# Mikata-Project/adcraft

Hardware: AMD Instinct MI355X
Metric: env-steps/sec (envs×keywords auctions/s) (higher is better)
Workload: dtype i32 cents + f32 (Philox4x32-7 u32); 1 GPU; cfg2: 4096 envs x 256 keywords per GPU, IMPLICIT keywords, mean_volume 128, cvr 0.8, no_vol_prob 0.0, drift False, budget non-binding, 60-step episodes with auto-reset; envs_per_gpu=4096, keywords=256, parallelism=env-sharded x1, collective=none (single GPU), weak_scaling_reference=also.cfg4.value of the N=1 --full line (same per-GPU shard as the N>1 runs)

## Files before the change

### adcraft_amd/_ffi.py

```python
import ctypes as C
import os

from . import build as _build

ADC_OK, ADC_EINVAL, ADC_EHIP, ADC_ENOMEM, ADC_ESTATE, ADC_ETYPE, ADC_ERCCL = 0, -1, -2, -3, -4, -5, -6
MODEL_IMPLICIT, MODEL_EXPLICIT, MODEL_IMPLICIT_GENERAL = 0, 1, 2
P_VOL_MEAN, P_VOL_STD, P_A, P_B, P_BCTR, P_SCTR, P_REV_MEAN, P_REV_STD, P_COUNT = range(9)
(BUF_PARAMS, BUF_BIDS, BUF_BUDGET, BUF_IMPRESSIONS, BUF_CLICKS, BUF_CONVERSIONS, BUF_COST, BUF_REVENUE, BUF_REWARD,
 BUF_CUM_PROFIT, BUF_DAYS, BUF_TERMINATED, BUF_TRUNCATED, BUF_METRIC_PROFIT, BUF_METRIC_SCALARS, BUF_FLAT_OBS,
 BUF_ROLLOUT_ACTION, BUF_ROLLOUT_LOGP, BUF_ROLLOUT_VALUE, BUF_ROLLOUT_REWARD, BUF_ROLLOUT_TERMINATED, BUF_ROLLOUT_TRUNCATED,
 BUF_ROLLOUT_OBS) = range(23)
MLP_TANH, MLP_RELU = 0, 1
ES_CENTERED_RANK, ES_RAW = 0, 1
ES_ADAM, ES_SGD = 0, 1
ROLLOUT_OBS = 1
PG_ADAM, PG_SGD = 0, 1
TD3_ADAM, TD3_SGD = 0, 1
PBT_PG, PBT_TD3 = 0, 1


class EngineError(RuntimeError):
    pass


# ... 161 lines not shown
        "adc_engine_set_env_drift": ([vp, vp], C.c_int),
        "adc_engine_get_rng_state": ([vp, vp, vp], C.c_int),
        "adc_engine_set_rng_state": ([vp, vp, vp], C.c_int),
        "adc_engine_get_episode_state": ([vp, vp, vp], C.c_int),
        "adc_engine_set_episode_state": ([vp, vp, vp], C.c_int),
        "adc_engine_step": ([vp, vp, vp, C.POINTER(StepOut)], C.c_int),
        "adc_engine_step_device": ([vp, vp, vp], C.c_int),
        "adc_engine_step_async": ([vp, vp, vp, C.POINTER(StepOut)], C.c_int),
        "adc_engine_step_flat_async": ([vp, vp, vp, vp, vp, vp], C.c_int),
        "adc_engine_wait": ([vp], C.c_int),
        "adc_engine_fetch": ([vp, C.POINTER(StepOut)], C.c_int),
        "adc_engine_out_offsets": ([vp, C.POINTER(C.c_size_t), C.POINTER(C.c_size_t)], C.c_int),
        "adc_engine_synchronize": ([vp], C.c_int),
        "adc_engine_step_flat": ([vp, vp, vp, vp, vp, vp], C.c_int),
        "adc_engine_step_replay": ([vp, vp, vp, C.POINTER(Tape), C.POINTER(StepOut)], C.c_int),
        "adc_engine_update_keywords": ([vp], C.c_int),
        "adc_engine_set_general_model": ([vp, i32, f32, i32], C.c_int),
        "adc_host_alloc": ([C.c_size_t, C.POINTER(vp)], C.c_int),
        "adc_host_free": ([vp], None),
        "adc_engine_device_buffer": ([vp, C.c_int, C.POINTER(vp), C.POINTER(C.c_size_t)], C.c_int),
        "adc_engine_stream": ([vp, C.POINTER(vp)], C.c_int),
        "adc_engine_sample_actions": ([vp, f32, f32, f32], C.c_int),
        "adc_engine_set_flat_actions_device": ([vp, vp], C.c_int),
        "adc_engine_flat_obs_enable": ([vp, C.c_int], C.c_int),
        "adc_engine_profile_enable": ([vp, C.c_int], C.c_int),
        "adc_engine_profile_sample_every": ([vp, C.c_int32], C.c_int),
        "adc_engine_profile_read": ([vp, vp, C.POINTER(i64)], C.c_int),
        "adc_engine_profile_records": ([vp, C.POINTER(i64)], C.c_int),
        "adc_engine_region_begin": ([vp], C.c_int),
        "adc_engine_region_end": ([vp, C.POINTER(f64)], C.c_int),
        "adc_engine_comm_stats": ([vp, C.POINTER(i64), C.POINTER(f64), C.POINTER(f64), C.c_int], C.c_int),
        "adc_engine_step_kernel_name": ([vp], C.c_char_p),
        "adc_engine_metrics_enable": ([vp, C.c_int], C.c_int),
        "adc_engine_metrics_reset": ([vp], C.c_int),
        "adc_engine_metrics_read": ([vp, vp, vp], C.c_int),
        "adc_engine_ideal_profit": ([vp, C.c_int, vp, C.c_int, vp], C.c_int),
        "adc_bid_curves_from_samples": ([C.c_int, vp, i32, vp, i32, vp, vp], C.c_int),
        "adc_engine_metrics_akncp_ncp": ([vp, f64, vp, vp], C.c_int),
        "adc_engine_bid_curves_contenders": ([vp, vp, vp, C.POINTER(i32)], C.c_int),
        "adc_engine_outcomes_replay": ([vp, i32, i32, vp, f32, i64, vp, vp, vp, vp, C.POINTER(i64), vp], C.c_int),
        "adc_engine_outcomes_replay_tape": ([vp, i32, vp, f32, C.POINTER(Tape), i64, vp, vp, vp, vp, C.POINTER(i64), vp], C.c_int),
        "adc_nth_price_auction": ([C.c_int, f64, vp, i32, i32, i32, i32, C.POINTER(i32), vp, vp], C.c_int),
        "adc_sigmoid": ([f64, f64, f64], f64),
        "adc_clamp": ([f64, f64, f64], f64),
        "adc_threshold_sigmoid": ([f64, f64, f64, f64], f64),
        "adc_sum_f64": ([vp, i64], f64),
        "adc_count_true": ([vp, i64], i64),
        "adc_nonneg_int_normal": ([f64, f64, u64, u64], u64),
        "adc_binomial": ([u64, f64, u64, u64], u64),
        "adc_cost_create": ([f64, i64, u64, u64, vp], C.c_int),
        "adc_auction_word_intervals": ([f32, f32, f32, f32, vp], C.c_int),
        "adc_auction_word_brackets": ([f32, f32, f32, f32, vp], C.c_int),
        "adc_check_win_brackets": ([i64, vp, vp, vp, vp, vp, vp, vp], i64),
        "adc_sample_random_keyword": ([C.c_uint64, C.c_uint32, C.c_uint32, vp], C.c_int),
        "adc_interp_act_host": ([f32, i32, f32, i32, C.c_double, C.c_double, C.c_double, vp, i32, i32, vp, vp, i32, vp, vp,
                                 C.c_double, vp, vp, vp, vp, vp], C.c_int),
        "adc_interp_key_host": ([f32], C.c_double),
        "adc_engine_mlp_init": ([vp, C.POINTER(MLPConfig), vp], C.c_int),
        "adc_engine_mlp_set_layer": ([vp, i32, i32, vp, vp], C.c_int),
        "adc_engine_mlp_set_norm": ([vp, vp, vp], C.c_int),
        "adc_engine_mlp_set_log_std": ([vp, vp], C.c_int),
        "adc_engine_mlp_set_deterministic": ([vp, i32], C.c_int),
        "adc_engine_mlp_act": ([vp, f32, vp], C.c_int),
        "adc_engine_mlp_step": ([vp, f32], C.c_int),
        "adc_engine_mlp_last": ([vp, vp, vp, vp, vp, vp], C.c_int),
        "adc_engine_mlp_bootstrap_value": ([vp, vp], C.c_int),
        "adc_engine_mlp_agent_state": ([vp, vp, vp], C.c_int),
        "adc_engine_rollout_enable": ([vp, i32, i32], C.c_int),
        "adc_engine_rollout_reset": ([vp], C.c_int),
        "adc_engine_rollout_fetch": ([vp, C.POINTER(i32), vp, vp, vp, vp, vp, vp, vp], C.c_int),
        "adc_engine_mlp_population": ([vp, i32, vp], C.c_int),
        "adc_engine_mlp_set_member_layer": ([vp, i32, i32, vp, vp], C.c_int),
        "adc_engine_mlp_param_count": ([vp, C.POINTER(i64)], C.c_int),
        "adc_engine_mlp_get_params": ([vp, vp], C.c_int),
        "adc_engine_mlp_get_member_params": ([vp, i32, vp], C.c_int),
        "adc_engine_mlp_learners": ([vp, i32], C.c_int),
        "adc_engine_mlp_set_learner_layer": ([vp, i32, i32, i32, vp, vp], C.c_int),
        "adc_engine_mlp_set_learner_log_std": ([vp, i32, vp], C.c_int),
        "adc_engine_mlp_get_learner_params": ([vp, i32, vp], C.c_int),
        "adc_engine_es_init": ([vp, C.POINTER(ESConfig)], C.c_int),
        "adc_engine_es_perturb": ([vp], C.c_int),
        "adc_engine_es_fitness": ([vp, vp], C.c_int),
        "adc_engine_es_update": ([vp, vp, C.POINTER(ESStats)], C.c_int),
        "adc_engine_es_state_get": ([vp, vp, vp, vp, C.POINTER(i64)], C.c_int),
        "adc_engine_es_state_set": ([vp, vp, vp, vp, i64], C.c_int),
        "adc_es_config_check": ([C.POINTER(ESConfig), C.POINTER(C.c_char_p)], C.c_int),
        "adc_es_noise_host": ([u64, C.c_uint32, C.c_uint32, i64, i64, vp], C.c_int),
        "adc_es_update_host": ([C.POINTER(ESConfig), u64, i32, i64, vp, i64, vp, vp, vp, vp], C.c_int),
        "adc_engine_pg_init": ([vp, C.POINTER(PGConfig)], C.c_int),
        "adc_engine_pg_param_count": ([vp, C.POINTER(i64)], C.c_int),
        "adc_engine_pg_advantages": ([vp], C.c_int),
        "adc_engine_pg_advantages_fetch": ([vp, vp, vp], C.c_int),
        "adc_engine_pg_minibatch": ([vp, i32, i32, C.POINTER(PGStats)], C.c_int),
        "adc_engine_pg_update": ([vp, i32, C.POINTER(PGStats)], C.c_int),
        "adc_engine_pg_state_get": ([vp, vp, vp, vp, C.POINTER(i64)], C.c_int),
        "adc_engine_pg_state_set": ([vp, vp, vp, vp, i64], C.c_int),
        "adc_pg_pop_config_check": ([C.POINTER(PGConfig), i32, i32, i32, C.POINTER(C.c_char_p)], C.c_int),
        "adc_engine_pg_pop_init": ([vp, C.POINTER(PGConfig), i32], C.c_int),
        "adc_engine_pg_pop_advantages": ([vp], C.c_int),
        "adc_engine_pg_pop_advantages_fetch": ([vp, vp, vp], C.c_int),
        "adc_engine_pg_pop_minibatch": ([vp, i32, C.POINTER(PGStats)], C.c_int),
        "adc_engine_pg_pop_update": ([vp, i32, C.POINTER(PGStats)], C.c_int),
        "adc_engine_pg_pop_state_get": ([vp, i32, vp, vp, vp, C.POINTER(i64)], C.c_int),
        "adc_engine_pg_pop_state_set": ([vp, i32, vp, vp, vp, i64], C.c_int),
        "adc_engine_pg_pop_set_config": ([vp, i32, C.POINTER(PGConfig)], C.c_int),
        "adc_engine_pg_pop_copy": ([vp, i32, i32], C.c_int),
# ... 141 lines not shown
```

### adcraft_amd/csrc/adc_law.h

```cpp
#pragma once
#include <stdint.h>

#if defined(__HIPCC__)
#include <hip/hip_runtime.h>
#define ADC_HD __host__ __device__ __forceinline__
#else
#include <math.h>
#define ADC_HD static inline
#endif

namespace adc {

enum Stage : uint32_t { ST_VOL = 0, ST_AUCTION = 1, ST_DRIFT = 2, ST_XPHANTOM = 3, ST_XREV = 4, ST_ACTION = 5, ST_METRIC = 6, ST_CONV = 7, ST_KEYGEN = 8, ST_AGENT = 9,
                        ST_GBIDDERS = 10, ST_GBID = 11, ST_GCLICK = 12, ST_INTERP = 13, ST_MLP = 14 };
constexpr int kTimesteps = 24;
constexpr int kVolumeMax = 1 << 20;
constexpr float kMoneyMaxCents = 1.0e9f;

struct U4 { uint32_t x, y, z, w; };

ADC_HD uint32_t xor3(uint32_t a, uint32_t b, uint32_t c)
{
#if defined(__HIP_DEVICE_COMPILE__)
    return __builtin_amdgcn_bitop3_b32(a, b, c, 0x96);
// ... 311 lines not shown
template <typename Tab>
ADC_HD float laplace_deviate_from_v(uint32_t v24, Tab tab)
{
    const uint32_t neg_mask = 0u - (v24 >> 23);
    const uint32_t mag = (v24 ^ neg_mask) & 0x007FFFFFu;
    const float e = neg_log_f24(fma32((float)mag, 2.0f, 1.0f), tab);
    return bits_to_float(xor_and(float_to_bits(-e), neg_mask, 0x80000000u));
}

template <typename Tab>
ADC_HD int32_t signed_cents_from_v(uint32_t v24, float loc, float scale, Tab tab)
{
    const float x = fma32(__builtin_fabsf(scale), laplace_deviate_from_v(v24, tab), loc);
    float c = __builtin_rintf(x * 100.0f);
    c = c < kMoneyMaxCents ? c : kMoneyMaxCents;
    c = c > -kMoneyMaxCents ? c : -kMoneyMaxCents;
    return (int32_t)c;
}

template <typename Tab>
ADC_HD int32_t competitor_cents_from_v(uint32_t v24, float loc, float scale, Tab tab)
{
    const float x = fma32(__builtin_fabsf(scale), laplace_deviate_from_v(v24, tab), loc);
    float c = __builtin_rintf(__builtin_fabsf(x) * 100.0f);
    c = c < kMoneyMaxCents ? c : kMoneyMaxCents;
    return (int32_t)c;
}

ADC_HD uint32_t auction_uniform24(uint32_t w, const AuctionLaw &a, bool &click)
{
    click = bernoulli32(w, a.t32);
    const uint32_t d = click ? w : w - a.t32;
    const uint32_t v = mulhi32(d, click ? a.m_click : a.m_noclick);
    return v < 0x00FFFFFFu ? v : 0x00FFFFFFu;
}

ADC_HD bool auction_wins(uint32_t w, int32_t bid_c, int32_t comp_c) { return bid_c > comp_c && w != 0xFFFFFFFFu; }

template <typename Tab>
ADC_HD int32_t auction_outcome_unless_top_word(uint32_t w, const AuctionLaw &a, float loc, float scale, Tab tab, bool &click)
{
    click = w < a.t32;
    const uint32_t d = click ? w : w - a.t32;
    const uint32_t v = mulhi32(d, click ? a.m_click : a.m_noclick);
    return competitor_cents_from_v(v < 0x00FFFFFFu ? v : 0x00FFFFFFu, loc, scale, tab);
}

ADC_HD int32_t auction_outcome(uint32_t w, const AuctionLaw &a, float loc, float scale, const LogTableEntry *tab, bool &click)
{
    return competitor_cents_from_v(auction_uniform24(w, a, click), loc, scale, tab);
}


ADC_HD uint32_t lower_bound_v(int32_t target, float loc, float scale, const LogTableEntry *tab)
{
    const float s = __builtin_fabsf(scale);
    const float x_t = ((float)target - 0.5f) * 0.01f;
    const float z_t = (x_t - loc) / s;
    const float e_t = __builtin_fabsf(z_t);
#if defined(__HIP_DEVICE_COMPILE__)
    float mag_f = __builtin_amdgcn_exp2f(fma32(e_t, -1.44269504f, 23.0f));
#else
    float mag_f = exp2f(fma32(e_t, -1.44269504f, 23.0f));
#endif
    mag_f = mag_f < 8388607.0f ? mag_f : 8388607.0f;
    mag_f = mag_f > 0.0f ? mag_f : 0.0f;
    const uint32_t mag = (uint32_t)mag_f;
    const uint32_t est = z_t < 0.0f ? mag : 0x00FFFFFFu - mag;
    float slack = mag_f * (6.0e-6f + 2.4e-7f * (__builtin_fabsf(x_t) + __builtin_fabsf(loc)) / s);
    slack = slack < 4194304.0f ? slack : 4194304.0f;
    const uint32_t half = 8u + (uint32_t)slack;
    uint32_t lo = est > half ? est - half : 0u;
    uint32_t hi = est + half < 0x01000000u ? est + half : 0x01000000u;
    if (lo > 0u && !(signed_cents_from_v(lo - 1u, loc, scale, tab) < target)) lo = 0u;
    if (hi < 0x01000000u && !(signed_cents_from_v(hi, loc, scale, tab) >= target)) hi = 0x01000000u;
    while (lo < hi) {
        const uint32_t mid = (lo + hi) >> 1;
        if (signed_cents_from_v(mid, loc, scale, tab) >= target) hi = mid;
        else lo = mid + 1u;
    }
    return lo;
}

ADC_HD uint64_t offset_reaching(uint32_t W, uint32_t m, uint64_t range)
{
    if (W == 0u) return 0ull;
    if (W > 0x00FFFFFFu || m == 0u) return range;
    const double q = ((double)W * 4294967296.0) / (double)m;
    if (!(q < (double)range)) return range;
    uint64_t d = (uint64_t)q;
    const uint64_t need = (uint64_t)W << 32;
    if (d * m >= need) { if (d > 0ull && (d - 1ull) * m >= need) d -= 1ull; }
    else { d += 1ull; if (d * m < need) d += 1ull; }
    return d < range ? d : range;
}

struct WinIntervals { uint32_t c_lo, c_w, n_lo, n_w; };

ADC_HD WinIntervals win_intervals(int32_t bid_c, float loc, float scale, uint64_t t_click, const AuctionLaw &law, const LogTableEntry *tab)
{
    const uint32_t w_lo = lower_bound_v(1 - bid_c, loc, scale, tab);
    const uint32_t w_hi = lower_bound_v(bid_c, loc, scale, tab);
    WinIntervals r{0u, 0u, 0u, 0u};
    if (!(w_lo < w_hi)) return r;
    const uint64_t top = 0xFFFFFFFFull;
    uint64_t a = offset_reaching(w_lo, law.m_click, t_click), b = offset_reaching(w_hi, law.m_click, t_click);
    b = b < top ? b : top;
    if (a < b) { r.c_lo = (uint32_t)a; r.c_w = (uint32_t)(b - a); }
    const uint64_t range_n = 4294967296ull - t_click;
    a = t_click + offset_reaching(w_lo, law.m_noclick, range_n);
    b = t_click + offset_reaching(w_hi, law.m_noclick, range_n);
    b = b < top ? b : top;
    if (a < b) { r.n_lo = (uint32_t)a; r.n_w = (uint32_t)(b - a); }
    return r;
}

struct WinBrackets { WinIntervals out, in; };
constexpr float kWordSlack = 4096.0f;

ADC_HD float fast_exp2(float x)
{
#if defined(__HIP_DEVICE_COMPILE__)
    return __builtin_amdgcn_exp2f(x);
#else
    return exp2f(x);
#endif
}
ADC_HD float fast_rcp(float x)
{
#if defined(__HIP_DEVICE_COMPILE__)
    return __builtin_amdgcn_rcpf(x);
#else
    return 1.0f / x;
#endif
}
ADC_HD float min_num(float a, float b) { return __builtin_fminf(a, b); }
ADC_HD float max_num(float a, float b) { return __builtin_fmaxf(a, b); }
ADC_HD uint32_t sat_sub(uint32_t a, uint32_t b)
{
#if defined(__clang__)
    return __builtin_elementwise_sub_sat(a, b);
#else
    return a > b ? a - b : 0u;
#endif
}
ADC_HD uint32_t to_word(float x)
{
#if defined(__HIP_DEVICE_COMPILE__)
    return (uint32_t)x;
#else
    return !(x > 0.0f) ? 0u : x >= 4294967296.0f ? 0xFFFFFFFFu : (uint32_t)x;
#endif
}

ADC_HD void lower_bound_estimate(float x_t, float loc, float inv_s, float &est, float &slack)
{
    const float z_t = (x_t - loc) * inv_s;
    const float e_t = __builtin_fabsf(z_t);
    const float mag = min_num(fast_exp2(fma32(e_t, -1.44269504f, 23.0f)), 8388607.0f);
    est = z_t < 0.0f ? mag : 16777215.0f - mag;
    const float rel = fma32(1.0e-6f, fma32(__builtin_fabsf(x_t) + __builtin_fabsf(loc), inv_s, e_t), 2.0e-5f);
    slack = min_num(fma32(mag, rel, 16.0f), 33554432.0f);
}

ADC_HD WinBrackets win_brackets(int32_t bid_c, float loc, float scale, float t_f)
{
    const float inv_s = fast_rcp(__builtin_fabsf(scale));
    const float bc = (float)bid_c;
    float lo, lo_s, hi, hi_s;
    lower_bound_estimate(fma32(bc, -0.01f, 0.005f), loc, inv_s, lo, lo_s);
    lower_bound_estimate(fma32(bc, 0.01f, -0.005f), loc, inv_s, hi, hi_s);
    const float lo_out = lo - lo_s, lo_in = lo + lo_s, hi_out = hi + hi_s, hi_in = hi - hi_s;
    const float a_c = max_num(t_f * 5.9604644775390625e-08f, 1.0f);
    const float a_n = max_num((4294967296.0f - t_f) * 5.9604644775390625e-08f, 1.0f);
    const float t_dn = t_f - kWordSlack, t_up = t_f + kWordSlack;
    WinBrackets r;
    const uint32_t c_lo_out = to_word(fma32(lo_out, a_c, -kWordSlack)), c_hi_out = to_word(min_num(fma32(hi_out, a_c, kWordSlack), t_f));
    const uint32_t c_lo_in = to_word(fma32(lo_in, a_c, kWordSlack)), c_hi_in = to_word(min_num(fma32(hi_in, a_c, -kWordSlack), t_f));
    const uint32_t n_lo_out = to_word(fma32(lo_out, a_n, t_dn)), n_hi_out = to_word(fma32(hi_out, a_n, t_up));
    const uint32_t n_lo_in = to_word(fma32(lo_in, a_n, t_up)), n_hi_in = to_word(fma32(hi_in, a_n, t_dn));
    r.out = WinIntervals{c_lo_out, sat_sub(c_hi_out, c_lo_out), n_lo_out, sat_sub(n_hi_out, n_lo_out)};
    r.in = WinIntervals{c_lo_in, sat_sub(c_hi_in, c_lo_in), n_lo_in, sat_sub(n_hi_in, n_lo_in)};
    return r;
}

ADC_HD void clicked_win_interval(int32_t bid_c, float loc, float scale, uint64_t t_click, const AuctionLaw &law, const LogTableEntry *tab,
                                 uint32_t &lo, uint32_t &width)
{
    lo = 0u;
    width = 0u;
    const uint32_t w_lo = lower_bound_v(1 - bid_c, loc, scale, tab), w_hi = lower_bound_v(bid_c, loc, scale, tab);
    if (!(w_lo < w_hi)) return;
    const uint64_t a = offset_reaching(w_lo, law.m_click, t_click);
    uint64_t b = offset_reaching(w_hi, law.m_click, t_click);
    b = b < 0xFFFFFFFFull ? b : 0xFFFFFFFFull;
    if (a < b) { lo = (uint32_t)a; width = (uint32_t)(b - a); }
}

ADC_HD int32_t revenue_cents_tab(uint32_t w, float mu, float sd, const NormTableEntry *tab)
{
    float x = fma32(sd, normal_tab(w, tab), mu);
    x = x > 0.01f ? x : 0.01f;
    return money_to_cents(x);
}

ADC_HD int32_t revenue_cents(uint32_t w, float mu, float sd)
{
    float x = fma32(sd, normal_from_word(w), mu);
    x = x > 0.01f ? x : 0.01f;
    return money_to_cents(x);
}

ADC_HD int32_t volume_from_word(uint32_t w, float mean, float sd, const NormTableEntry *tab)
{
    float x = fma32(sd, normal_tab(w, tab), mean);
    x = x > 0.0f ? x : 0.0f;
    x = x < (float)kVolumeMax ? x : (float)kVolumeMax;
    const float t = __builtin_truncf(x);
    return (int32_t)t + ((x - t) >= 0.5f ? 1 : 0);
}

ADC_HD int64_t bid_to_cents(float bid)
{
    double c = __builtin_rint((double)bid * 100.0);
    if (!(c >= 1.0)) c = 1.0;
    if (c > 1.0e9) c = 1.0e9;
    return (int64_t)c;
}
ADC_HD int32_t bid_to_cents_i32(float bid)
{
    double c = __builtin_rint((double)bid * 100.0);
    if (!(c >= 1.0)) c = 1.0;
    if (c > 1.0e9) c = 1.0e9;
    return (int32_t)c;
}
ADC_HD int64_t budget_to_cents(float budget)
{
    double c = __builtin_rint((double)budget * 100.0);
    if (!(c > -9.0e15)) c = -9.0e15;
    if (c > 9.0e15) c = 9.0e15;
    return (int64_t)c;
}

ADC_HD double cents_to_dollars_f64(int cents)
// ... 272 lines not shown
```

### adcraft_amd/csrc/adc_shims.cpp

```cpp
#include <algorithm>
#include <cmath>
#include <cstdint>
#include <thread>
#include <vector>

#include "../../include/adcraft_engine.h"
#include "adc_law.h"
#include "adc_interp.h"
#include "adc_mlp.h"
#include "adc_es.h"
#include "adc_pg.h"
#include "adc_td3.h"
#include "adc_pbt.h"
#include "adc_norm.h"
#include "adc_rew_norm.h"
#include "adc_td3_norm.h"

#define ADC_EXPORT extern "C" __attribute__((visibility("default")))

ADC_EXPORT double adc_sigmoid(double x, double s, double t) { return 1.0 / (1.0 + std::exp(-s * (x - t))); }

ADC_EXPORT double adc_clamp(double x, double lo, double hi) { return x < lo ? lo : (x > hi ? hi : x); }

ADC_EXPORT double adc_threshold_sigmoid(double p, double impression_thresh, double impression_bid_intercept,
// ... 71 lines not shown
{
    if (!out4) return ADC_EINVAL;
    const adc::LogTableEntry *table = host_log_table();
    const adc::AuctionLaw law = adc::make_auction_law(buyside_ctr);
    const adc::WinIntervals r = adc::win_intervals((int32_t)adc::bid_to_cents(bid), cost_loc, cost_scale,
                                                   adc::bernoulli_threshold(buyside_ctr), law, table);
    out4[0] = r.c_lo; out4[1] = r.c_w; out4[2] = r.n_lo; out4[3] = r.n_w;
    return ADC_OK;
}

ADC_EXPORT int adc_auction_word_brackets(float bid, float cost_loc, float cost_scale, float buyside_ctr, uint32_t *out8)
{
    if (!out8) return ADC_EINVAL;
    const adc::WinBrackets b = adc::win_brackets((int32_t)adc::bid_to_cents(bid), cost_loc, cost_scale, adc::bernoulli_threshold_f32(buyside_ctr));
    out8[0] = b.out.c_lo; out8[1] = b.out.c_w; out8[2] = b.out.n_lo; out8[3] = b.out.n_w;
    out8[4] = b.in.c_lo; out8[5] = b.in.c_w; out8[6] = b.in.n_lo; out8[7] = b.in.n_w;
    return ADC_OK;
}

static inline bool interval_inside(uint32_t a_lo, uint32_t a_w, uint32_t b_lo, uint32_t b_w)
{
    if (a_w == 0u) return true;
    return b_w != 0u && a_lo >= b_lo && (uint64_t)a_lo + a_w <= (uint64_t)b_lo + b_w;
}

ADC_EXPORT int64_t adc_check_win_brackets(int64_t n, const float *bid, const float *cost_loc, const float *cost_scale, const float *buyside_ctr,
                                          const uint32_t *brackets8, int64_t *first_bad, double *ambiguous_words)
{
    if (n < 0 || !bid || !cost_loc || !cost_scale || !buyside_ctr) return -1;
    const adc::LogTableEntry *table = host_log_table();
    int64_t bad = 0, first = -1;
    double amb = 0.0;
    for (int64_t i = 0; i < n; ++i) {
        const int32_t bid_c = (int32_t)adc::bid_to_cents(bid[i]);
        const adc::AuctionLaw law = adc::make_auction_law(buyside_ctr[i]);
        const adc::WinIntervals x = adc::win_intervals(bid_c, cost_loc[i], cost_scale[i], adc::bernoulli_threshold(buyside_ctr[i]), law, table);
        adc::WinBrackets b;
        if (brackets8) {
            const uint32_t *p = brackets8 + 8 * i;
            b.out = adc::WinIntervals{p[0], p[1], p[2], p[3]};
            b.in = adc::WinIntervals{p[4], p[5], p[6], p[7]};
        } else {
            b = adc::win_brackets(bid_c, cost_loc[i], cost_scale[i], adc::bernoulli_threshold_f32(buyside_ctr[i]));
        }
        const bool ok = interval_inside(b.in.c_lo, b.in.c_w, x.c_lo, x.c_w) && interval_inside(x.c_lo, x.c_w, b.out.c_lo, b.out.c_w) &&
                        interval_inside(b.in.n_lo, b.in.n_w, x.n_lo, x.n_w) && interval_inside(x.n_lo, x.n_w, b.out.n_lo, b.out.n_w) &&
                        (uint64_t)b.out.c_lo + b.out.c_w <= 0xFFFFFFFFull && (uint64_t)b.out.n_lo + b.out.n_w <= 0xFFFFFFFFull;
        if (!ok) { if (first < 0) first = i; ++bad; }
        amb += ((double)b.out.c_w - (double)b.in.c_w) + ((double)b.out.n_w - (double)b.in.n_w);
    }
    if (first_bad) *first_bad = first;
    if (ambiguous_words) *ambiguous_words = amb;
    return bad;
}

ADC_EXPORT int adc_sample_random_keyword(uint64_t key, uint32_t keyword, uint32_t serial, float *out8)
{
    if (!out8) return ADC_EINVAL;
    adc::generate_explicit_keyword(key, keyword, serial, out8);
    return ADC_OK;
}

ADC_EXPORT int adc_explicit_curve_host(uint64_t key, uint32_t tick, int32_t keyword, int32_t n_samples, float impression_thresh, float a,
                                       float b, const double *bid_grid, int32_t n_bids, double *ir_out, double *cpc_out, double *z_mid2_out)
{
    if (n_samples <= 0 || n_samples > (1 << 20) || keyword < 0 || n_bids < 0 || (n_bids > 0 && (!bid_grid || !ir_out || !cpc_out)))
        return ADC_EINVAL;
    std::vector<float> z((size_t)n_samples);
    for (int32_t i = 0; i < n_samples; i += 4) {
        const adc::U4 w = adc::draw(key, (uint32_t)(i / 4), adc::ST_METRIC, (uint32_t)keyword, tick);
        const uint32_t ws[4] = {w.x, w.y, w.z, w.w};
        for (int j = 0; j < 4 && i + j < n_samples; ++j) z[(size_t)(i + j)] = adc::normal_from_word(ws[j]);
    }
    std::sort(z.begin(), z.end());
    const float z_lo = z[(size_t)((n_samples - 1) / 2)], z_hi = z[(size_t)(n_samples / 2)];
    if (z_mid2_out) { z_mid2_out[0] = z_lo; z_mid2_out[1] = z_hi; }
    for (int32_t i = 0; i < n_bids; ++i) {
        double mu, sigma;
        adc::explicit_cost_law(bid_grid[i], mu, sigma);
        const adc::CurvePoint q = adc::explicit_curve_point(impression_thresh, a, b, z_lo, z_hi, bid_grid[i], mu, sigma);
        ir_out[i] = q.ir;
        cpc_out[i] = q.cpc;
    }
    return ADC_OK;
}

ADC_EXPORT double adc_interp_key_host(float bid) { return adc::interp_key(bid); }

ADC_EXPORT int adc_interp_act_host(float ave_rpc, int32_t n_rpc, float ave_sctr, int32_t n_sctr, double max_observed, double threshold,
                                   double bid_step, const double *grid, int32_t n_bids, int32_t n_clk, const uint16_t *clk_cent,
                                   const float *clk_ave, int32_t n_cpc, const uint16_t *cpc_cent, const double *cpc_ave, double u,
                                   double *margin_out, double *cost_out, double *bid_out, int32_t *index_out,
                                   double *mass_out)
{
    if (n_bids < 1 || n_bids > adc::kInterpMaxBids || !grid || n_clk < 0 || n_cpc < 0 || n_clk > adc::kInterpCents ||
        n_cpc > n_clk || (n_clk > 0 && (!clk_cent || !clk_ave)) || (n_cpc > 0 && (!cpc_cent || !cpc_ave)) || !bid_out || !index_out)
        return ADC_EINVAL;
    for (int i = 0; i < n_clk; ++i)
        if (clk_cent[i] < 1 || clk_cent[i] > adc::kInterpCents || (i > 0 && clk_cent[i] <= clk_cent[i - 1])) return ADC_EINVAL;
    for (int i = 0; i < n_cpc; ++i)
        if (cpc_cent[i] < 1 || cpc_cent[i] > adc::kInterpCents || (i > 0 && cpc_cent[i] <= cpc_cent[i - 1])) return ADC_EINVAL;
    const adc::InterpSeries<float> clk{clk_cent, clk_ave, 1, n_clk};
    const adc::InterpSeries<double> cpc{cpc_cent, cpc_ave, 1, n_cpc};
    double cpc_right = 0.0;
    for (int i = 0; i < n_cpc; ++i) cpc_right = (i == 0 || cpc_ave[i] > cpc_right) ? cpc_ave[i] : cpc_right;
    const double erpc = adc::interp_erpc(ave_rpc, n_rpc, ave_sctr, n_sctr);
// ... 812 lines not shown
```

### adcraft_amd/csrc/parts/kernel_exact_rows.inc

```
#ifdef ADC_EXP_TIMING
#define DBG_T() wall_clock64()
#define DBG_ADD(i, x) dbg[i] += (x)
#else
#define DBG_T() 0ull
#define DBG_ADD(i, x) (void)0
#endif
constexpr int kRowsBlock = 256;
#ifndef ADC_ROWS_MIN_BLOCKS
#define ADC_ROWS_MIN_BLOCKS 4
#endif
constexpr int kRowsMinBlocks = ADC_ROWS_MIN_BLOCKS;
#ifndef ADC_ROWS_MIN_BLOCKS_ONE
#define ADC_ROWS_MIN_BLOCKS_ONE 6
#endif
constexpr int kRowsMinBlocksOne = ADC_ROWS_MIN_BLOCKS_ONE;
constexpr int kRowsMaxK = 2048;
constexpr int kRowsRing = 128;

struct CellStat {
    unsigned int wins, clicks, first;
    unsigned int mask;
    unsigned long long total;
    double sum_d;
    unsigned long long q4;
// ... 637 lines not shown
    __syncthreads();
    if (tid == 0 && !handed) {
        long long profit_c = 0;
        for (int i = 0; i < BLOCK / kWave; ++i) profit_c += rs.wave_part[i];
        exact_pass_epilogue(v, env, hint_in, few_clicks, was_binding, bound_t);
        step_tail(v, env, tick, true, profit_c, 0.0);
    }
    __syncthreads();
    if (tid == 0) rs.cur = (int)gridDim.x + atomicAdd(&v.flag_next[parity], 1);
    __syncthreads();
    fi = rs.cur;
    DBG_ADD(4, 1);
  }
#ifdef ADC_EXP_TIMING
  if (tid == 0) for (int i = 0; i < 8; ++i) atomicAdd(&g_dbg[i], dbg[i]);
#endif
}


#ifdef ADC_EXP_TIMING
__device__ unsigned long long g_rest_phase[20];
#define RDBG_ADD(slot, val) do { if (tid == 0) atomicAdd(&g_rest_phase[slot], (unsigned long long)(val)); } while (0)
#define RDBG_MAX(slot, val) do { if (tid == 0) atomicMax(&g_rest_phase[slot], (unsigned long long)(val)); } while (0)
#else
#define RDBG_ADD(slot, val) (void)0
#define RDBG_MAX(slot, val) (void)0
#endif
constexpr int kRestMaxK = 1024;
struct RestShared {
    long long wave_part[kRowsMaxWaves];
    long long f_R;
    double f_rd;
    int stop_cell;
    int cur;
    int mark_cnt[1][kRowsMaxWaves];
};
constexpr int kRestMarks = 1024;
__host__ __device__ inline size_t rest_lds_bytes(int K) { return (size_t)K * (adc::kTimesteps * 2 + 2 * 8 + 3 * 4); }

struct RestLaws { adc::WinIntervals iv, cheap; adc::AuctionLaw law; float loc, scale; int vol, j_from; };
__device__ __forceinline__ RestLaws rest_laws(const View &v, const float *__restrict__ bids, int env, int K, const RestState &st, int k)
{
    RestLaws L;
    const size_t o = (size_t)env * K + k;
    L.vol = (int)v.rest_counts[o].w;
    int32_t n_unused;
    if (st.row < adc::kTimesteps) adc::cell_range(L.vol, st.row, L.j_from, n_unused);
    else L.j_from = L.vol;
    const int bid_c = (int)adc::bid_to_cents(bids[o]);
    L.loc = param_at(v, ADC_P_A, env, k);
    L.scale = param_at(v, ADC_P_B, env, k);
    const float bctr = param_at(v, ADC_P_BCTR, env, k);
    L.law = adc::make_auction_law(bctr);
    L.iv = adc::win_intervals(bid_c, L.loc, L.scale, adc::bernoulli_threshold(bctr), L.law, g_log_table);
    const int cheap_bid = min(bid_c, (int)(st.R < 0x3FFFFFFFll ? (st.R > 0 ? st.R : 0) : 0x3FFFFFFFll) + 1);
    L.cheap = adc::win_brackets(cheap_bid, L.loc, L.scale, adc::bernoulli_threshold_f32(bctr)).out;
    return L;
}
__device__ __forceinline__ unsigned int rest_count_wins(uint64_t key, uint32_t tick, int K, int k, const RestLaws &L, int a, int b, unsigned short *table)
{
    unsigned int w_count = 0u;
    int last_cw = -1;
    auto one = [&](uint32_t word, int j) {
        const bool cw = (word - L.iv.c_lo) < L.iv.c_w;
        w_count += (unsigned int)(cw | ((word - L.iv.n_lo) < L.iv.n_w));
        if (table && cw && (word - L.cheap.c_lo) < L.cheap.c_w) {
            const int s24 = L.vol / adc::kTimesteps, first24 = L.vol - (adc::kTimesteps - 1) * s24;
            const int row = j < first24 ? 0 : min(1 + (j - first24) / max(s24, 1), adc::kTimesteps - 1);
            const int row_start = row == 0 ? 0 : first24 + (row - 1) * s24;
            if (last_cw < row_start) {
                bool click_bit;
                const int comp = adc::auction_outcome(word, L.law, L.loc, L.scale, g_log_table, click_bit);
                table[row * K + k] = (unsigned short)min(comp, 0xFFFE);
            }
        }
        last_cw = cw ? j : last_cw;
    };
    for (int q = a >> 2; 4 * q < b; ++q) {
        const adc::U4 w = adc::draw(key, (uint32_t)q, adc::ST_AUCTION, (uint32_t)k, tick);
        if (4 * q >= a && 4 * q + 4 <= b) {
            one(w.x, 4 * q); one(w.y, 4 * q + 1); one(w.z, 4 * q + 2); one(w.w, 4 * q + 3);
        } else {
#pragma unroll
            for (int h = 0; h < 4; ++h) {
                const int j = 4 * q + h;
                if (j >= a && j < b) one(h == 0 ? w.x : h == 1 ? w.y : h == 2 ? w.z : w.w, j);
            }
        }
    }
    return w_count;
}

constexpr int kRestPassBlocks = 6;
#ifndef ADC_REST_FRESH_BLOCKS
#define ADC_REST_FRESH_BLOCKS 5
#endif
constexpr int kRestFreshBlocks = ADC_REST_FRESH_BLOCKS;
template <bool PASS_ONLY, bool FRESH = false, int BLOCK = kRowsBlock>
__global__ __launch_bounds__(BLOCK, BLOCK == 512 ? 6 : FRESH ? kRestFreshBlocks : PASS_ONLY ? kRestPassBlocks : 5) void k_step_rest_of_day(View v, const float *__restrict__ bids, int parity)
{
    static_assert(PASS_ONLY || !FRESH, "the at-once variant hands its marks to k_rest_walk");
    static_assert(BLOCK == kRowsBlock || (PASS_ONLY && !FRESH), "wider workgroups: the plain pass only");
    extern __shared__ __align__(16) unsigned char rest_raw[];
    __shared__ RestShared sh;
    const int K = v.K;
    unsigned long long *const a_cost = reinterpret_cast<unsigned long long *>(rest_raw);
    unsigned long long *const a_rev = a_cost + K;
// ... 582 lines not shown
```

### include/adcraft_engine.h

```cpp
#ifndef ADCRAFT_ENGINE_H
#define ADCRAFT_ENGINE_H

#include <stddef.h>
#include <stdint.h>

#ifdef __cplusplus
extern "C" {
#endif

#define ADC_ABI_VERSION 5
#define ADC_STREAM_REVISION 5

typedef enum adc_status {
    ADC_OK = 0,
    ADC_EINVAL = -1,
    ADC_EHIP = -2,
    ADC_ENOMEM = -3,
    ADC_ESTATE = -4,
    ADC_ETYPE = -5,
    ADC_ERCCL = -6
} adc_status;

typedef enum adc_model {
    ADC_MODEL_IMPLICIT = 0,
// ... 446 lines not shown
int adc_pg_gae_norm_host(const adc_pg_config *cfg, int32_t days, int32_t num_envs, const float *reward_tn, const uint8_t *terminated_tn,
                         const uint8_t *truncated_tn, const float *value_tn, const float *bootstrap_n, const float *scale_n, float clip,
                         float *adv_tn, float *ret_tn);

typedef struct adc_td3_norm_config {
    uint32_t struct_size;
    int32_t observations, rewards;
    int32_t per_member;
    double obs_min_std;
    int64_t obs_count_cap;
    double rew_min_std;
    int64_t rew_count_cap;
    float rew_clip;
} adc_td3_norm_config;
int adc_td3_norm_config_check(const adc_td3_norm_config *cfg, const char **message);
int adc_engine_td3_norm_init(adc_engine *e, const adc_td3_norm_config *cfg);
int adc_engine_td3_norm_update(adc_engine *e, int64_t *samples);
int adc_engine_td3_norm_state_get(adc_engine *e, int32_t member, int64_t *obs_count, double *obs_mean_d, double *obs_m2_d, float *shift_d, float *scale_d,
                                  int64_t *rew_count, double *rew_mean, double *rew_m2, float *rew_scale);
int adc_engine_td3_norm_state_set(adc_engine *e, int32_t member, int64_t obs_count, const double *obs_mean_d, const double *obs_m2_d, const float *shift_d,
                                  const float *scale_d, int64_t rew_count, double rew_mean, double rew_m2, float rew_scale);
int adc_engine_td3_norm_returns_get(adc_engine *e, double *g_n);
int adc_engine_td3_norm_returns_set(adc_engine *e, const double *g_n);
int adc_engine_td3_norm_copy(adc_engine *e, const int32_t *src_of_member_m);
int adc_td3_norm_obs_host(const adc_td3_norm_config *cfg, int64_t S, int32_t D, const float *x_sd, int64_t *count, double *mean_d, double *m2_d,
                          float *shift_d, float *scale_d);
int adc_td3_norm_rew_host(const adc_td3_norm_config *cfg, int32_t days, int32_t num_envs, const float *gamma_n, const float *reward_tn,
                          const uint8_t *terminated_tn, const uint8_t *truncated_tn, int64_t *count, double *mean, double *m2, float *scale,
                          double *carry_n);
int adc_td3_y_norm_host(const adc_td3_config *td3, int32_t count, const float *r_b, const uint8_t *done_b, const float *q_b, float scale, float clip,
                        float *y_b);

int adc_engine_outcomes_replay(adc_engine *e, int32_t env, int32_t steps_back, const float *bids_k, float budget, int64_t capacity,
                               int32_t *keyword, int32_t *timestep, double *cost, double *revenue, int64_t *count, int32_t *share_volume_k);
int adc_engine_outcomes_replay_tape(adc_engine *e, int32_t env, const float *bids_k, float budget, const adc_tape *tape, int64_t capacity,
                                    int32_t *keyword, int32_t *timestep, double *cost, double *revenue, int64_t *count, int32_t *share_volume_k);

int adc_nth_price_auction(int device_id, double bid, const double *other_bids, int32_t n_auctions, int32_t n_bidders,
                          int32_t n, int32_t num_winners, int32_t *impressions, int32_t *placements, double *costs);

double adc_sigmoid(double x, double s, double t);
double adc_clamp(double x, double lo, double hi);
double adc_threshold_sigmoid(double p, double impression_thresh,
                             double impression_bid_intercept, double impression_slope);
double adc_sum_f64(const double *x, int64_t n);
int64_t adc_count_true(const uint8_t *x, int64_t n);
uint64_t adc_nonneg_int_normal(double mean, double std, uint64_t seed, uint64_t counter);
uint64_t adc_binomial(uint64_t n, double p, uint64_t seed, uint64_t counter);
int adc_cost_create(double x, int64_t n, uint64_t seed, uint64_t counter, double *out_n);
int adc_auction_word_intervals(float bid, float cost_loc, float cost_scale, float buyside_ctr, uint32_t *out4);
int adc_auction_word_brackets(float bid, float cost_loc, float cost_scale, float buyside_ctr, uint32_t *out8);
int64_t adc_check_win_brackets(int64_t n, const float *bid, const float *cost_loc, const float *cost_scale, const float *buyside_ctr,
                               const uint32_t *brackets8, int64_t *first_bad, double *ambiguous_words);
int adc_sample_random_keyword(uint64_t key, uint32_t keyword, uint32_t serial, float *out8);
int adc_explicit_curve_host(uint64_t key, uint32_t tick, int32_t keyword, int32_t n_samples, float impression_thresh, float a, float b,
                            const double *bid_grid, int32_t n_bids, double *ir_out, double *cpc_out, double *z_mid2_out);
int adc_interp_act_host(float ave_rpc, int32_t num_rpc_obs, float ave_sctr, int32_t num_sctr_obs, double max_observed,
                        double profit_acquisition_threshold, double bid_step, const double *allowed_bids, int32_t n_bids,
                        int32_t n_clicks, const uint16_t *clicks_cent, const float *ave_clicks, int32_t n_cpc, const uint16_t *cpc_cent,
                        const double *ave_cpc, double u, double *margin_out, double *cost_out, double *bid_out, int32_t *index_out,
                        double *mass_out);
double adc_interp_key_host(float bid);
int adc_mlp_act_host(const adc_mlp_config *cfg, int32_t num_keywords, const float *obs_d, const float *const *policy_w,
                     const float *const *policy_b, const float *const *value_w, const float *const *value_b, const float *shift_d,
                     const float *scale_d, const float *log_std_a, const float *normals_a, uint64_t agent_key, uint32_t tick,
                     float budget_override, float *mean_a, float *log_std_out_a, float *action_a, float *logp, float *value,
                     float *bids_k, float *budget);
int adc_es_config_check(const adc_es_config *cfg, const char **message);
int adc_es_noise_host(uint64_t seed, uint32_t pair, uint32_t generation, int64_t p0, int64_t n, float *eps_n);
int adc_es_update_host(const adc_es_config *cfg, uint64_t seed, int32_t members, int64_t n_params, const double *fitness_m, int64_t generation,
                       float *theta_p, float *m_p, float *v_p, float *grad_p);
int adc_pg_config_check(const adc_pg_config *cfg, const char **message);
int adc_pg_gae_host(const adc_pg_config *cfg, int32_t days, int32_t num_envs, const float *reward_tn, const uint8_t *terminated_tn,
                    const uint8_t *truncated_tn, const float *value_tn, const float *bootstrap_n, float *adv_tn, float *ret_tn);
int adc_pg_param_count_host(const adc_mlp_config *mlp, int32_t num_keywords, int64_t *count);
int adc_pg_grad_host(const adc_mlp_config *mlp, int32_t num_keywords, const adc_pg_config *cfg, const float *theta_q, int64_t count,
                     const float *obs_sd, const float *action_sa, const float *logp_old_s, const float *adv_s, const float *ret_s,
                     const float *value_old_s, float *grad_q, double *sums10, adc_pg_stats *stats);
int adc_pg_step_host(const adc_pg_config *cfg, int64_t n_params, int64_t steps_taken, const float *grad_q, float *theta_q, float *m_q,
                     float *v_q);
int adc_td3_config_check(const adc_td3_config *cfg, const char **message);
int adc_td3_param_counts_host(const adc_mlp_config *mlp, int32_t num_keywords, const adc_td3_config *cfg, int64_t *actor_p, int64_t *critic_qc);
int adc_td3_batch_indices_host(uint64_t seed, int64_t update, int64_t size, int32_t count, int32_t *idx_b);
int adc_td3_target_host(const adc_mlp_config *mlp, int32_t num_keywords, const adc_td3_config *cfg, uint64_t seed, int64_t update,
                        const float *theta_target_p, const float *psi_target_q, const float *shift_a, const float *scale_a, int32_t count,
                        const float *x2_bd, const float *r_b, const uint8_t *done_b, float *y_b);
int adc_td3_critic_grad_host(const adc_mlp_config *mlp, int32_t num_keywords, const adc_td3_config *cfg, const float *psi_q,
                             const float *shift_a, const float *scale_a, int32_t count, const float *x_bd, const float *a_ba, const float *y_b,
                             float *grad_q, double *sums6);
int adc_td3_actor_grad_host(const adc_mlp_config *mlp, int32_t num_keywords, const adc_td3_config *cfg, const float *theta_p,
                            const float *psi_q, const float *shift_a, const float *scale_a, int32_t count, const float *x_bd, float *grad_p,
                            double *sums2);
int adc_td3_polyak_host(float tau, int64_t n, const float *param_n, float *target_n);
int adc_pbt_fitness_host(int32_t days, int32_t num_envs, int32_t members, const float *reward_tn, double *fitness_m);
int adc_pbt_plan_host(const adc_pbt_config *cfg, uint64_t seed, int32_t members, int64_t round, const double *fitness_m, double *smoothed_m,
                      int32_t *rank_m, int32_t *src_m, uint32_t *bits_m);
int adc_pbt_explore_host(const adc_pbt_config *cfg, int32_t kind, uint32_t bits, const float *donor_hp8, const float *own_hp8, float *out_hp8);
int adc_mlp_config_check(const adc_mlp_config *cfg, int32_t num_keywords, const char **message);
float adc_mlp_math_host(int32_t fn, float x);
int64_t adc_mlp_math_sweep_host(int32_t fn, float lo, float hi, double *out3, int64_t *violations4);
uint64_t adc_mlp_agent_key_host(uint64_t seed);
uint64_t adc_mlp_default_agent_key_host(uint64_t engine_seed, uint64_t global_env_id);
int adc_debug_philox_device(int device_id, int64_t n, const uint32_t *ctr4, const uint32_t *key2, uint32_t *out4);
int adc_debug_chain_device(int device_id, double r0, int64_t n, const double *x, double *out2);
int adc_debug_walk_stats(adc_engine *e, int64_t stats[4], int reset);
int adc_debug_direct_days(adc_engine *e, int64_t *env_days, int reset);
// ... 8 lines not shown
```

Measured before the change: 6.399 billion keyword-steps/s.

## Replace lower-bound bisection with Newton-estimated window and wave-uniform fallback

The inverse-CDF lower bound for the Laplace cost law now gets a first estimate from exp2, then takes one Newton-style correction using the table slope. It checks three neighbouring words and falls back to a neighbour probe or the full bisection only when some lane in the wavefront needs it. Win-interval computation evaluates the low and high bounds side by side. The exact-rows kernel explicitly keeps the old per-bound path, and host shims are added to validate the new path. This cuts the per-lane binary-search iterations and the divergence they cause, at the cost of more code and a ballot-gated fallback.

```diff
diff --git a/adcraft_amd/_ffi.py b/adcraft_amd/_ffi.py
--- a/adcraft_amd/_ffi.py
+++ b/adcraft_amd/_ffi.py
@@ -237,6 +237,9 @@
         "adc_auction_word_intervals": ([f32, f32, f32, f32, vp], C.c_int),
         "adc_auction_word_brackets": ([f32, f32, f32, f32, vp], C.c_int),
         "adc_check_win_brackets": ([i64, vp, vp, vp, vp, vp, vp, vp], i64),
+        "adc_lower_bound_v_host": ([i64, vp, vp, vp, vp, vp], C.c_int),
+        "adc_lower_bound_v_bisect_host": ([i64, vp, vp, vp, vp, vp], C.c_int),
+        "adc_win_intervals_host": ([i64, vp, vp, vp, vp, i32, vp, vp], C.c_int),
         "adc_sample_random_keyword": ([C.c_uint64, C.c_uint32, C.c_uint32, vp], C.c_int),
         "adc_interp_act_host": ([f32, i32, f32, i32, C.c_double, C.c_double, C.c_double, vp, i32, i32, vp, vp, i32, vp, vp,
                                  C.c_double, vp, vp, vp, vp, vp], C.c_int),
diff --git a/adcraft_amd/csrc/adc_law.h b/adcraft_amd/csrc/adc_law.h
--- a/adcraft_amd/csrc/adc_law.h
+++ b/adcraft_amd/csrc/adc_law.h
@@ -387,7 +387,26 @@
 }
 
 
-ADC_HD uint32_t lower_bound_v(int32_t target, float loc, float scale, const LogTableEntry *tab)
+ADC_HD float fast_exp2(float x)
+{
+#if defined(__HIP_DEVICE_COMPILE__)
+    return __builtin_amdgcn_exp2f(x);
+#else
+    return exp2f(x);
+#endif
+}
+ADC_HD float fast_rcp(float x)
+{
+#if defined(__HIP_DEVICE_COMPILE__)
+    return __builtin_amdgcn_rcpf(x);
+#else
+    return 1.0f / x;
+#endif
+}
+ADC_HD float min_num(float a, float b) { return __builtin_fminf(a, b); }
+ADC_HD float max_num(float a, float b) { return __builtin_fmaxf(a, b); }
+
+ADC_HD uint32_t lower_bound_v_bisect(int32_t target, float loc, float scale, const LogTableEntry *tab, bool *whole_range = nullptr)
 {
     const float s = __builtin_fabsf(scale);
     const float x_t = ((float)target - 0.5f) * 0.01f;
@@ -407,14 +426,128 @@
     const uint32_t half = 8u + (uint32_t)slack;
     uint32_t lo = est > half ? est - half : 0u;
     uint32_t hi = est + half < 0x01000000u ? est + half : 0x01000000u;
+    const uint32_t lo_w = lo, hi_w = hi;
     if (lo > 0u && !(signed_cents_from_v(lo - 1u, loc, scale, tab) < target)) lo = 0u;
     if (hi < 0x01000000u && !(signed_cents_from_v(hi, loc, scale, tab) >= target)) hi = 0x01000000u;
+    if (whole_range) *whole_range = lo != lo_w || hi != hi_w;
     while (lo < hi) {
         const uint32_t mid = (lo + hi) >> 1;
         if (signed_cents_from_v(mid, loc, scale, tab) >= target) hi = mid;
         else lo = mid + 1u;
     }
     return lo;
+}
+
+template <typename Tab>
+ADC_HD float laplace_deviate_and_slope(uint32_t v24, Tab tab, float &dz_dv)
+{
+    const uint32_t neg_mask = 0u - (v24 >> 23);
+    const uint32_t mag = (v24 ^ neg_mask) & 0x007FFFFFu;
+    const uint32_t bits = float_to_bits(fma32((float)mag, 2.0f, 1.0f));
+    const float ef = (float)((int)(bits >> 23) - 151);
+    const uint32_t mant = bits & 0x007FFFFFu;
+    const LogTableEntry t = log_entry(tab, mant >> 15);
+    float r = fma32(t.slope, (float)(mant & 0x7FFFu), t.value);
+    r = fma32(ef, -2.12194440e-4f, r);
+    r = fma32(ef, 0.693359375f, r);
+    dz_dv = t.slope * bits_to_float((278u - (bits >> 23)) << 23);
+    return bits_to_float(xor_and(float_to_bits(r), neg_mask, 0x80000000u));
+}
+
+ADC_HD int32_t lower_bound_window(int32_t target, float loc, float scale, const LogTableEntry *tab)
+{
+    const float tf = (float)target;
+    const float xs = (tf - 0.5f) * 0.01f;
+    const float ulp = bits_to_float(float_to_bits(xs) & 0x7F800000u) * 1.1920928955078125e-07f;
+    const bool ge0 = __builtin_rintf(xs * 100.0f) >= tf;
+    const float x1 = ge0 ? xs - ulp : xs + ulp;
+    const bool ge1 = __builtin_rintf(x1 * 100.0f) >= tf;
+    const float below = ge0 ? (ge1 ? x1 - ulp : x1) : (ge1 ? xs : x1);
+    const float inv_s = fast_rcp(__builtin_fabsf(scale));
+    const float z_t = fma32(ulp, 0.5f, below - loc) * inv_s;
+    const float mag_f = max_num(min_num(fast_exp2(fma32(__builtin_fabsf(z_t), -1.44269504f, 23.0f)), 8388607.0f), 0.0f);
+    const uint32_t mag = (uint32_t)mag_f;
+    const uint32_t est = z_t < 0.0f ? mag : 0x00FFFFFFu - mag;
+    float dz_dv;
+    const float z_e = laplace_deviate_and_slope(est, tab, dz_dv);
+    const float step = __builtin_rintf((z_t - z_e) * fast_rcp(dz_dv));
+    const int32_t b = (int32_t)est + (int32_t)max_num(min_num(step, 16777216.0f), -16777216.0f) - 1;
+    return b < -1 ? -1 : b > 0x00FFFFFF ? 0x00FFFFFF : b;
+}
+
+ADC_HD bool bound_reached(int32_t i, int32_t target, float loc, float scale, const LogTableEntry *tab)
+{
+    const uint32_t v = (uint32_t)(i < 0 ? 0 : i > 0x00FFFFFF ? 0x00FFFFFF : i);
+    const bool g = signed_cents_from_v(v, loc, scale, tab) >= target;
+    return i < 0 ? false : i > 0x00FFFFFF ? true : g;
+}
+
+ADC_HD bool any_lane(bool c)
+{
+#if defined(__HIP_DEVICE_COMPILE__)
+    return __builtin_amdgcn_ballot_w64(c) != 0ull;
+#else
+    return c;
+#endif
+}
+
+enum BoundStage : int { kBoundAccepted = 0, kBoundNeighbour = 1, kBoundBisected = 2 };
+
+struct BoundTrial { int32_t b; bool g0, g1, g2; };
+
+ADC_HD BoundTrial bound_trial(int32_t b, int32_t target, float loc, float scale, const LogTableEntry *tab)
+{
+    return BoundTrial{b, bound_reached(b, target, loc, scale, tab), bound_reached(b + 1, target, loc, scale, tab),
+                      bound_reached(b + 2, target, loc, scale, tab)};
+}
+ADC_HD bool bound_open(const BoundTrial &t) { return t.g0 || !t.g2; }
+ADC_HD uint32_t bound_accepted(const BoundTrial &t) { return (uint32_t)(t.b + (t.g1 ? 1 : 2)); }
+
+ADC_HD uint32_t lower_bound_finish(const BoundTrial &t, int32_t target, float loc, float scale, const LogTableEntry *tab, int &stage)
+{
+    uint32_t v = bound_accepted(t);
+    bool open = bound_open(t);
+    if (open) {
+        const bool down = t.g0;
+        const int32_t from = t.b + (down ? -3 : 3);
+        const bool h0 = bound_reached(from, target, loc, scale, tab), h1 = bound_reached(from + 1, target, loc, scale, tab),
+                   h2 = bound_reached(from + 2, target, loc, scale, tab);
+        const int first = h0 ? 0 : h1 ? 1 : h2 ? 2 : 3;
+        if (down ? first != 0 : first != 3) { v = (uint32_t)(from + first); open = false; stage = kBoundNeighbour; }
+    }
+    if (any_lane(open)) {
+        if (open) { v = lower_bound_v_bisect(target, loc, scale, tab); stage = kBoundBisected; }
+    }
+    return v;
+}
+
+ADC_HD uint32_t lower_bound_v_staged(int32_t target, float loc, float scale, const LogTableEntry *tab, int &stage)
+{
+    const BoundTrial t = bound_trial(lower_bound_window(target, loc, scale, tab), target, loc, scale, tab);
+    stage = kBoundAccepted;
+    if (any_lane(bound_open(t))) return lower_bound_finish(t, target, loc, scale, tab, stage);
+    return bound_accepted(t);
+}
+
+ADC_HD uint32_t lower_bound_v(int32_t target, float loc, float scale, const LogTableEntry *tab)
+{
+    int stage;
+    return lower_bound_v_staged(target, loc, scale, tab, stage);
+}
+
+ADC_HD void lower_bound_pair(int32_t bid_c, float loc, float scale, const LogTableEntry *tab, uint32_t &w_lo, uint32_t &w_hi, int &stage)
+{
+    const int32_t b_lo = lower_bound_window(1 - bid_c, loc, scale, tab), b_hi = lower_bound_window(bid_c, loc, scale, tab);
+    const BoundTrial t_lo = bound_trial(b_lo, 1 - bid_c, loc, scale, tab), t_hi = bound_trial(b_hi, bid_c, loc, scale, tab);
+    w_lo = bound_accepted(t_lo);
+    w_hi = bound_accepted(t_hi);
+    stage = kBoundAccepted;
+    if (any_lane(bound_open(t_lo) || bound_open(t_hi))) {
+        int s_lo = kBoundAccepted, s_hi = kBoundAccepted;
+        w_lo = lower_bound_finish(t_lo, 1 - bid_c, loc, scale, tab, s_lo);
+        w_hi = lower_bound_finish(t_hi, bid_c, loc, scale, tab, s_hi);
+        stage = s_lo > s_hi ? s_lo : s_hi;
+    }
 }
 
 ADC_HD uint64_t offset_reaching(uint32_t W, uint32_t m, uint64_t range)
@@ -432,10 +565,8 @@
 
 struct WinIntervals { uint32_t c_lo, c_w, n_lo, n_w; };
 
-ADC_HD WinIntervals win_intervals(int32_t bid_c, float loc, float scale, uint64_t t_click, const AuctionLaw &law, const LogTableEntry *tab)
-{
-    const uint32_t w_lo = lower_bound_v(1 - bid_c, loc, scale, tab);
-    const uint32_t w_hi = lower_bound_v(bid_c, loc, scale, tab);
+ADC_HD WinIntervals win_intervals_of_bounds(uint32_t w_lo, uint32_t w_hi, uint64_t t_click, const AuctionLaw &law)
+{
     WinIntervals r{0u, 0u, 0u, 0u};
     if (!(w_lo < w_hi)) return r;
     const uint64_t top = 0xFFFFFFFFull;
@@ -450,27 +581,23 @@
     return r;
 }
 
+template <bool SIDE_BY_SIDE = true>
+ADC_HD WinIntervals win_intervals(int32_t bid_c, float loc, float scale, uint64_t t_click, const AuctionLaw &law, const LogTableEntry *tab)
+{
+    uint32_t w_lo, w_hi;
+    if constexpr (SIDE_BY_SIDE) {
+        int stage;
+        lower_bound_pair(bid_c, loc, scale, tab, w_lo, w_hi, stage);
+    } else {
+        w_lo = lower_bound_v(1 - bid_c, loc, scale, tab);
+        w_hi = lower_bound_v(bid_c, loc, scale, tab);
+    }
+    return win_intervals_of_bounds(w_lo, w_hi, t_click, law);
+}
+
 struct WinBrackets { WinIntervals out, in; };
 constexpr float kWordSlack = 4096.0f;
 
-ADC_HD float fast_exp2(float x)
-{
-#if defined(__HIP_DEVICE_COMPILE__)
-    return __builtin_amdgcn_exp2f(x);
-#else
-    return exp2f(x);
-#endif
-}
-ADC_HD float fast_rcp(float x)
-{
-#if defined(__HIP_DEVICE_COMPILE__)
-    return __builtin_amdgcn_rcpf(x);
-#else
-    return 1.0f / x;
-#endif
-}
-ADC_HD float min_num(float a, float b) { return __builtin_fminf(a, b); }
-ADC_HD float max_num(float a, float b) { return __builtin_fmaxf(a, b); }
 ADC_HD uint32_t sat_sub(uint32_t a, uint32_t b)
 {
 #if defined(__clang__)
@@ -524,7 +651,9 @@
 {
     lo = 0u;
     width = 0u;
-    const uint32_t w_lo = lower_bound_v(1 - bid_c, loc, scale, tab), w_hi = lower_bound_v(bid_c, loc, scale, tab);
+    uint32_t w_lo, w_hi;
+    int stage;
+    lower_bound_pair(bid_c, loc, scale, tab, w_lo, w_hi, stage);
     if (!(w_lo < w_hi)) return;
     const uint64_t a = offset_reaching(w_lo, law.m_click, t_click);
     uint64_t b = offset_reaching(w_hi, law.m_click, t_click);
diff --git a/adcraft_amd/csrc/adc_shims.cpp b/adcraft_amd/csrc/adc_shims.cpp
--- a/adcraft_amd/csrc/adc_shims.cpp
+++ b/adcraft_amd/csrc/adc_shims.cpp
@@ -147,6 +147,72 @@
     if (first_bad) *first_bad = first;
     if (ambiguous_words) *ambiguous_words = amb;
     return bad;
+}
+
+template <typename F>
+static void shim_parallel_for(int64_t n, F body)
+{
+    const int T = n < 4096 ? 1 : 8;
+    std::vector<std::thread> threads;
+    for (int t = 0; t < T; ++t) threads.emplace_back([=]() { body(n * t / T, n * (t + 1) / T); });
+    for (auto &th : threads) th.join();
+}
+
+ADC_EXPORT int adc_lower_bound_v_host(int64_t n, const int32_t *target, const float *loc, const float *scale, uint32_t *v_out, uint8_t *stage_out)
+{
+    if (n < 0 || (n > 0 && (!target || !loc || !scale || !v_out))) return ADC_EINVAL;
+    const adc::LogTableEntry *table = host_log_table();
+    shim_parallel_for(n, [=](int64_t i0, int64_t i1) {
+        for (int64_t i = i0; i < i1; ++i) {
+            int stage = 0;
+            v_out[i] = adc::lower_bound_v_staged(target[i], loc[i], scale[i], table, stage);
+            if (stage_out) stage_out[i] = (uint8_t)stage;
+        }
+    });
+    return ADC_OK;
+}
+
+ADC_EXPORT int adc_lower_bound_v_bisect_host(int64_t n, const int32_t *target, const float *loc, const float *scale, uint32_t *v_out,
+                                             uint8_t *whole_range_out)
+{
+    if (n < 0 || (n > 0 && (!target || !loc || !scale || !v_out))) return ADC_EINVAL;
+    const adc::LogTableEntry *table = host_log_table();
+    shim_parallel_for(n, [=](int64_t i0, int64_t i1) {
+        for (int64_t i = i0; i < i1; ++i) {
+            bool whole = false;
+            v_out[i] = adc::lower_bound_v_bisect(target[i], loc[i], scale[i], table, &whole);
+            if (whole_range_out) whole_range_out[i] = whole ? 1 : 0;
+        }
+    });
+    return ADC_OK;
+}
+
+ADC_EXPORT int adc_win_intervals_host(int64_t n, const int32_t *bid_c, const float *cost_loc, const float *cost_scale, const float *buyside_ctr,
+                                      int32_t bisect, uint32_t *out4, uint8_t *stage_out)
+{
+    if (n < 0 || (n > 0 && (!bid_c || !cost_loc || !cost_scale || !buyside_ctr || !out4))) return ADC_EINVAL;
+    const adc::LogTableEntry *table = host_log_table();
+    shim_parallel_for(n, [=](int64_t i0, int64_t i1) {
+        for (int64_t i = i0; i < i1; ++i) {
+            const adc::AuctionLaw law = adc::make_auction_law(buyside_ctr[i]);
+            const uint64_t t_click = adc::bernoulli_threshold(buyside_ctr[i]);
+            uint32_t w_lo, w_hi;
+            int stage = 0;
+            if (bisect) {
+                bool a = false, b = false;
+                w_lo = adc::lower_bound_v_bisect(1 - bid_c[i], cost_loc[i], cost_scale[i], table, &a);
+                w_hi = adc::lower_bound_v_bisect(bid_c[i], cost_loc[i], cost_scale[i], table, &b);
+                stage = (a || b) ? 1 : 0;
+            } else {
+                adc::lower_bound_pair(bid_c[i], cost_loc[i], cost_scale[i], table, w_lo, w_hi, stage);
+            }
+            const adc::WinIntervals r = adc::win_intervals_of_bounds(w_lo, w_hi, t_click, law);
+            uint32_t *o = out4 + 4 * i;
+            o[0] = r.c_lo; o[1] = r.c_w; o[2] = r.n_lo; o[3] = r.n_w;
+            if (stage_out) stage_out[i] = (uint8_t)stage;
+        }
+    });
+    return ADC_OK;
 }
 
 ADC_EXPORT int adc_sample_random_keyword(uint64_t key, uint32_t keyword, uint32_t serial, float *out8)
diff --git a/adcraft_amd/csrc/parts/kernel_exact_rows.inc b/adcraft_amd/csrc/parts/kernel_exact_rows.inc
--- a/adcraft_amd/csrc/parts/kernel_exact_rows.inc
+++ b/adcraft_amd/csrc/parts/kernel_exact_rows.inc
@@ -713,7 +713,7 @@
     L.scale = param_at(v, ADC_P_B, env, k);
     const float bctr = param_at(v, ADC_P_BCTR, env, k);
     L.law = adc::make_auction_law(bctr);
-    L.iv = adc::win_intervals(bid_c, L.loc, L.scale, adc::bernoulli_threshold(bctr), L.law, g_log_table);
+    L.iv = adc::win_intervals<false>(bid_c, L.loc, L.scale, adc::bernoulli_threshold(bctr), L.law, g_log_table);
     const int cheap_bid = min(bid_c, (int)(st.R < 0x3FFFFFFFll ? (st.R > 0 ? st.R : 0) : 0x3FFFFFFFll) + 1);
     L.cheap = adc::win_brackets(cheap_bid, L.loc, L.scale, adc::bernoulli_threshold_f32(bctr)).out;
     return L;
diff --git a/include/adcraft_engine.h b/include/adcraft_engine.h
--- a/include/adcraft_engine.h
+++ b/include/adcraft_engine.h
@@ -522,6 +522,11 @@
 int adc_auction_word_brackets(float bid, float cost_loc, float cost_scale, float buyside_ctr, uint32_t *out8);
 int64_t adc_check_win_brackets(int64_t n, const float *bid, const float *cost_loc, const float *cost_scale, const float *buyside_ctr,
                                const uint32_t *brackets8, int64_t *first_bad, double *ambiguous_words);
+int adc_lower_bound_v_host(int64_t n, const int32_t *target_n, const float *loc_n, const float *scale_n, uint32_t *v_n, uint8_t *stage_n);
+int adc_lower_bound_v_bisect_host(int64_t n, const int32_t *target_n, const float *loc_n, const float *scale_n, uint32_t *v_n,
+                                  uint8_t *whole_range_n);
+int adc_win_intervals_host(int64_t n, const int32_t *bid_cents_n, const float *cost_loc_n, const float *cost_scale_n,
+                           const float *buyside_ctr_n, int32_t bisect, uint32_t *out4_n, uint8_t *stage_n);
 int adc_sample_random_keyword(uint64_t key, uint32_t keyword, uint32_t serial, float *out8);
 int adc_explicit_curve_host(uint64_t key, uint32_t tick, int32_t keyword, int32_t n_samples, float impression_thresh, float a, float b,
                             const double *bid_grid, int32_t n_bids, double *ir_out, double *cpc_out, double *z_mid2_out);
```

Result: faster. 6.558 billion keyword-steps/s (median of 6 runs) (+2.5%).
